# yurimjeon1892/EFGH

Hardware: AMD Instinct MI355X
Metric: frame-pairs/sec EFGHNet fwd+bwd (384x1280 RGB + 64x2048 range), whole job (higher is better)
Workload: dtype f32; 1 GPU; BASELINE.json configs[2]: EFGHNet fwd+bwd with efghloss + gradient all-reduce + fused Adam, synthetic 384x1280 RGB + 131072-point sweep, batch=8 per GPU, random-init weights; global_batch=8, points=131072, parallelism=dp1

## Files before the change

efgh_amd/csrc/wino.hip:

```cpp
#include "common.h"
#include <type_traits>


namespace {

typedef float f32x16 __attribute__((ext_vector_type(16)));

__device__ __attribute__((aligned(16))) float g_zero_page[16];

constexpr int TM = 64, TN = 64, KC = 16, LD = KC;

struct WinoArgs {
    const float *A; long long lda; int C;
    int B, H, W, TW;
    const float *U; int N;
    long long Mt;
    const float *bias, *scale, *shift, *residual; long long ldr;
    int act; float slope;
    float *out; long long ldo;
    float *stats;
    unsigned nbx;
    int smode;
    const float *bn_raw; long long bn_ldraw;
    const float *bn_y; long long bn_ldy;
    const float *bn_psc, *bn_psh, *bn_mean, *bn_invstd;
    int bn_act; float bn_slope;
};

template <bool BNM, bool HPOOL = false>
__global__ void __launch_bounds__(256, 2) k_wino43(const WinoArgs p) {
    __shared__ __attribute__((aligned(16))) float Vs[6 * TM * LD];
    __shared__ __attribute__((aligned(16))) float Us[6 * TN * LD];
    __shared__ long long tpix[TM];
    __shared__ int tcnt[TM];

    const int tid = threadIdx.x, lane = tid & 63, wave = tid >> 6;
    const int wm = wave >> 1, wn = wave & 1, l31 = lane & 31, lh = lane >> 5;
    const unsigned nbx = p.nbx, nblk = gridDim.x;
    const unsigned q8 = nblk >> 3, r8 = nblk & 7, xcd = blockIdx.x & 7, within = blockIdx.x >> 3;
    const unsigned lin = (xcd < r8 ? xcd * (q8 + 1) : r8 * (q8 + 1) + (xcd - r8) * q8) + within;
    const unsigned tile_m = lin / nbx, tile_n = lin - tile_m * nbx;
    const long long m0 = (long long)tile_m * TM;
    const int n0 = tile_n * TN;
    if (m0 >= p.Mt) return;

    const int st = tid >> 2, cq = (tid & 3) * 4;
    const int cqs = ((tid & 3) ^ ((st >> 2) & 3)) * 4;
    long long pix0 = 0;
    unsigned cmask = 0, rmask = 0;
    {
        const long long t = m0 + st;
        if (t < p.Mt) {
            const int xt = (int)(t % p.TW); const long long r = t / p.TW;
            const int y = (int)(r % p.H); const long long b = r / p.H;
            const int x0 = 4 * xt - 1;
#pragma unroll
            for (int q = 0; q < 6; ++q) if ((unsigned)(x0 + q) < (unsigned)p.W) cmask |= 1u << q;
#pragma unroll
            for (int kh = 0; kh < 3; ++kh) if ((unsigned)(y + kh - 1) < (unsigned)p.H) rmask |= 1u << kh;
            pix0 = (b * p.H + y) * p.W + x0;
        }
    }
    if (tid < TM) {
        const long long t = m0 + tid;
        long long o = -1; int cnt = 0;
        if (t < p.Mt) {
            const int xt = (int)(t % p.TW); const long long r = t / p.TW;
            o = r * p.W + 4 * xt;
            cnt = p.W - 4 * xt; cnt = cnt > 4 ? 4 : cnt;
            if (HPOOL) {
                const int wp = p.W >> 1;
                o = r * wp + 2 * xt;
                cnt = wp - 2 * xt; cnt = cnt > 2 ? 2 : cnt;
                if (cnt <= 0) { o = -1; cnt = 0; }
            }
        }
        tpix[tid] = o; tcnt[tid] = cnt;
    }
    const long long ustride = (long long)p.N * KC;
    const float *ubase = p.U + (long long)(n0 + st) * KC + cq;
// ... 48 lines not shown
                v4.e = q42 - q31;                                                                    \
                v5.e = 4.f * d1 - 5.f * d3 + d5;                                                     \
            }
            EFGH_BT(x) EFGH_BT(y) EFGH_BT(z) EFGH_BT(w)
#undef EFGH_BT
#define EFGH_ST(a, vv, uu)                                                                            \
            *reinterpret_cast<float4 *>(&Vs[(a * TM + st) * LD + cqs]) = vv;                         \
            *reinterpret_cast<float4 *>(&Us[(a * TN + st) * LD + cqs]) = uu;
            EFGH_ST(0, v0, ru0) EFGH_ST(1, v1, ru1) EFGH_ST(2, v2, ru2) EFGH_ST(3, v3, ru3) EFGH_ST(4, v4, ru4) EFGH_ST(5, v5, ru5)
#undef EFGH_ST
        }
        __syncthreads();
        const bool more = ch + 1 < nchunks;
        if (more) EFGH_CHUNK_ADDR(ch + 1)
        {
            const int sw = (l31 >> 2) & 3, q0 = ((2 * lh) ^ sw) * 4, q1 = ((2 * lh + 1) ^ sw) * 4;
            const float *va = &Vs[(wm * 32 + l31) * LD];
            const float *ub = &Us[(wn * 32 + l31) * LD];
            float4 fa[2][2], fb[2][2];
            fa[0][0] = *reinterpret_cast<const float4 *>(va + q0); fa[0][1] = *reinterpret_cast<const float4 *>(va + q1);
            fb[0][0] = *reinterpret_cast<const float4 *>(ub + q0); fb[0][1] = *reinterpret_cast<const float4 *>(ub + q1);
#pragma unroll
            for (int a = 0; a < 6; ++a) {
                const int cur = a & 1, nxt = cur ^ 1;
                if (a < 5) {
                    fa[nxt][0] = *reinterpret_cast<const float4 *>(va + (a + 1) * TM * LD + q0);
                    fa[nxt][1] = *reinterpret_cast<const float4 *>(va + (a + 1) * TM * LD + q1);
                    fb[nxt][0] = *reinterpret_cast<const float4 *>(ub + (a + 1) * TN * LD + q0);
                    fb[nxt][1] = *reinterpret_cast<const float4 *>(ub + (a + 1) * TN * LD + q1);
                }
                if (more) {
                    if (a == 0) EFGH_LOAD_PAIR(0, ra0, ru0)
                    if (a == 1) EFGH_LOAD_PAIR(1, ra1, ru1)
                    if (a == 2) EFGH_LOAD_PAIR(2, ra2, ru2)
                    if (a == 3) EFGH_LOAD_PAIR(3, ra3, ru3)
                    if (a == 4) EFGH_LOAD_PAIR(4, ra4, ru4)
                    if (a == 5) EFGH_LOAD_PAIR(5, ra5, ru5)
                }
                __builtin_amdgcn_sched_barrier(0);
                acc[a] = __builtin_amdgcn_mfma_f32_32x32x2f32(fa[cur][0].x, fb[cur][0].x, acc[a], 0, 0, 0);
                acc[a] = __builtin_amdgcn_mfma_f32_32x32x2f32(fa[cur][0].y, fb[cur][0].y, acc[a], 0, 0, 0);
                acc[a] = __builtin_amdgcn_mfma_f32_32x32x2f32(fa[cur][0].z, fb[cur][0].z, acc[a], 0, 0, 0);
                acc[a] = __builtin_amdgcn_mfma_f32_32x32x2f32(fa[cur][0].w, fb[cur][0].w, acc[a], 0, 0, 0);
                acc[a] = __builtin_amdgcn_mfma_f32_32x32x2f32(fa[cur][1].x, fb[cur][1].x, acc[a], 0, 0, 0);
                acc[a] = __builtin_amdgcn_mfma_f32_32x32x2f32(fa[cur][1].y, fb[cur][1].y, acc[a], 0, 0, 0);
                acc[a] = __builtin_amdgcn_mfma_f32_32x32x2f32(fa[cur][1].z, fb[cur][1].z, acc[a], 0, 0, 0);
                acc[a] = __builtin_amdgcn_mfma_f32_32x32x2f32(fa[cur][1].w, fb[cur][1].w, acc[a], 0, 0, 0);
                __builtin_amdgcn_sched_barrier(0);
            }
        }
        __syncthreads();
    }

    float *ssum = Vs, *ssq = Vs + 2 * TN;
    const int coll = wn * 32 + l31, col = n0 + coll;
    const float bi = p.bias ? p.bias[col] : 0.f;
    const float sc = p.scale ? p.scale[col] : 1.f;
    const float sf = p.shift ? p.shift[col] : 0.f;
    float s1 = 0.f, s2 = 0.f;
    constexpr bool bnm = BNM;
    float b_psc = 0.f, b_psh = 0.f, b_mu = 0.f, b_is = 0.f;
    if (bnm) {
        if (!p.bn_y) { b_psc = p.bn_psc[col]; b_psh = p.bn_psh[col]; }
        b_mu = p.bn_mean[col]; b_is = p.bn_invstd[col];
    }
    const float neg = p.act == 1 ? 0.f : (p.act == 2 ? p.slope : 1.f);
    auto rows = [&](auto res_c, auto full_c) {
        constexpr bool RES = decltype(res_c)::value, FULL = decltype(full_c)::value;
#pragma unroll
        for (int r = 0; r < 16; ++r) {
            const int rl = wm * 32 + (r & 3) + 8 * (r >> 2) + 4 * lh;
            const long long opix = tpix[rl];
            const int cnt = FULL ? 4 : tcnt[rl];
            if (!FULL && opix < 0) continue;
            float *op = p.out + opix * p.ldo + col;
            float rv[4] = {0.f, 0.f, 0.f, 0.f};
            if (RES) {
                const float *rp = p.residual + opix * p.ldr + col;
#pragma unroll
                for (int i = 0; i < 4; ++i) if (FULL || i < cnt) rv[i] = rp[i * p.ldr];
            }
            const float m0_ = acc[0][r], m1 = acc[1][r], m2 = acc[2][r], m3 = acc[3][r], m4 = acc[4][r], m5 = acc[5][r];
            const float s12 = m1 + m2, d12 = m1 - m2, s34 = m3 + m4, d34 = m3 - m4;
            const float yv[4] = {m0_ + s12 + s34, d12 + 2.f * d34, s12 + 4.f * s34, d12 + 8.f * d34 + m5};
            if (HPOOL) {
                float w[4];
#pragma unroll
                for (int i = 0; i < 4; ++i) { float v = yv[i] + bi; v = v * sc + sf; w[i] = act_neg(v, neg); }
                st_out(op, fmaxf(w[0], w[1]));
                if (FULL || cnt > 1) st_out(op + p.ldo, fmaxf(w[2], w[3]));
                continue;
            }
#pragma unroll
            for (int i = 0; i < 4; ++i) {
                if (!FULL && i >= cnt) continue;
                float v = yv[i] + bi;
                if (!bnm) { s1 += v; s2 = fmaf(v, v, s2); }
                v = v * sc + sf;
                if (RES) v += rv[i];
                v = act_neg(v, neg);
                st_out(op + i * p.ldo, v);
                if (bnm) {
                    const float rw = p.bn_raw[(opix + i) * p.bn_ldraw + col];
                    const float yy = p.bn_y ? p.bn_y[(opix + i) * p.bn_ldy + col] : rw * b_psc + b_psh;
                    const float g = p.bn_act == 1 ? (yy > 0.f ? v : 0.f) : p.bn_act == 2 ? (yy > 0.f ? v : v * p.bn_slope) : v;
                    s1 += g; s2 += g * ((rw - b_mu) * b_is);
                }
            }
        }
    };
    const bool full = m0 + TM <= p.Mt && (p.W & 3) == 0;
    if (p.residual) {
        if (full) rows(std::true_type{}, std::true_type{});
        else rows(std::true_type{}, std::false_type{});
    } else {
        if (full) rows(std::false_type{}, std::true_type{});
        else rows(std::false_type{}, std::false_type{});
    }
    if (p.stats) {
        s1 += __shfl_xor(s1, 32); s2 += __shfl_xor(s2, 32);
        if (lh == 0) { ssum[wm * TN + coll] = s1; ssq[wm * TN + coll] = s2; }
        __syncthreads();
        if (tid < TN) {
            p.stats[((long long)tile_m * 2 + 0) * p.N + n0 + tid] = ssum[tid] + ssum[TN + tid];
            p.stats[((long long)tile_m * 2 + 1) * p.N + n0 + tid] = ssq[tid] + ssq[TN + tid];
        }
    }
}

__global__ void k_wino_pack(const float *__restrict__ Wp, float *__restrict__ U, int N, int C) {
    const long long total = 3LL * C * N;
    for (long long i = (long long)blockIdx.x * blockDim.x + threadIdx.x; i < total; i += (long long)gridDim.x * blockDim.x)
        wino_pack_item(Wp, U, N, C, i);
}

constexpr int TT = 16;

struct WinoWArgs {
    const float *A; long long lda; int C;
    const float *G; long long ldg; int N;
    int B, H, W, TW;
    long long Mt; long long tchunk;
    float *S;
    unsigned kt, nt;
};

constexpr int WR_WAVES = 12;

__global__ void __launch_bounds__(64 * WR_WAVES, 1) k_wino_wgrad_rows(const WinoWArgs p, int strips, int chunks, int rh, int ct) {
    __shared__ __attribute__((aligned(16))) float Gs[6 * TT * 64];
    __shared__ __attribute__((aligned(16))) float Vr[3][6 * TT * 64];
    const int tid = threadIdx.x, lane = tid & 63, wave = __builtin_amdgcn_readfirstlane(tid >> 6);
    const int kg = wave >> 2, wn = (wave >> 1) & 1, wc = wave & 1, l31 = lane & 31, lh = lane >> 5;
    const int unit = blockIdx.x, strip = unit % strips, ur = unit / strips, chk = ur % chunks;
    const long long b = ur / chunks;
    const int y0 = chk * rh, y1 = y0 + rh < p.H ? y0 + rh : p.H;
    const int c0 = (blockIdx.y % ct) * 64, n0 = (blockIdx.y / ct) * 64;
    if (y0 >= y1) return;
    const int role = wave >> 2, st = tid & 255, ts = st >> 4, q4 = (st & 15) * 4;
    const int xt = strip * TT + ts, x0 = 4 * xt - 1, xg = 4 * xt;
    const bool tv = xt < p.TW;
    const float *zpage = g_zero_page;
    float4 r0, r1, r2, r3, r4, r5;
    auto load_x = [&](int r) {
        const bool rok = tv && (unsigned)r < (unsigned)p.H;
        const float *xrow = p.A + (((b * p.H + r) * p.W + x0) * p.lda + c0 + q4);
#define EFGH_LDX(q, dst) dst = *reinterpret_cast<const float4 *>((rok && (unsigned)(x0 + q) < (unsigned)p.W) ? xrow + (long long)q * p.lda : zpage);
        EFGH_LDX(0, r0) EFGH_LDX(1, r1) EFGH_LDX(2, r2) EFGH_LDX(3, r3) EFGH_LDX(4, r4) EFGH_LDX(5, r5)
#undef EFGH_LDX
    };
    auto load_g = [&](int r) {
        const float *grow = p.G + (((b * p.H + r) * p.W + xg) * p.ldg + n0 + q4);
#define EFGH_LDG(i, dst) dst = *reinterpret_cast<const float4 *>((tv && (xg + i) < p.W) ? grow + (long long)i * p.ldg : zpage);
        EFGH_LDG(0, r0) EFGH_LDG(1, r1) EFGH_LDG(2, r2) EFGH_LDG(3, r3)
#undef EFGH_LDG
    };
    auto stage_x = [&](float *V) {
        float4 v0, v1, v2, v3, v4, v5;
#define EFGH_TR(e)                                                                                    \
        {                                                                                            \
// ... 60 lines not shown
            for (int s8 = 0; s8 < 8; ++s8) { fg[0][s8] = gp[s8 * 128]; fv[0][s8] = vp[s8 * 128]; }
#pragma unroll
            for (int a = 0; a < 6; ++a) {
                const int cur = a & 1, nxt = cur ^ 1;
                if (a < 5) {
#pragma unroll
                    for (int s8 = 0; s8 < 8; ++s8) {
                        fg[nxt][s8] = gp[(a + 1) * TT * 64 + s8 * 128];
                        fv[nxt][s8] = vp[(a + 1) * TT * 64 + s8 * 128];
                    }
                }
#pragma unroll
                for (int s8 = 0; s8 < 8; ++s8)
                    acc[a] = __builtin_amdgcn_mfma_f32_32x32x2f32(fg[cur][s8], fv[cur][s8], acc[a], 0, 0, 0);
            }
        }
        __syncthreads();
        s0 = s0 == 2 ? 0 : s0 + 1;
    }
    const long long K3 = 3LL * p.C;
    float *sb = p.S + (((long long)unit * 3) * p.N + n0 + wn * 32) * K3 + kg * p.C + c0 + wc * 32 + l31;
    const long long plane = (long long)p.N * K3;
#pragma unroll
    for (int r = 0; r < 16; ++r) {
        const int nl = (r & 3) + 8 * (r >> 2) + 4 * lh;
        const float s0 = acc[0][r], s1 = acc[1][r], s2 = acc[2][r], s3 = acc[3][r], s4 = acc[4][r], s5 = acc[5][r];
        sb[nl * K3] = s0 + s1 + s2 + s3 + s4;
        sb[plane + nl * K3] = (s1 - s2) + 2.f * (s3 - s4);
        sb[2 * plane + nl * K3] = (s1 + s2) + 4.f * (s3 + s4) + s5;
    }
}

__global__ void k_wino_wgrad_finish3(const float *__restrict__ S, float *__restrict__ dWp, int N, int C, long long on, long long oc,
                                     long long ot, int Nr, int Cr, int accumulate) {
    const long long K3 = 3LL * C, total = (long long)N * K3;
    for (long long i = (long long)blockIdx.x * blockDim.x + threadIdx.x; i < total; i += (long long)gridDim.x * blockDim.x) {
        const int kc = (int)(i % K3); const long long n = i / K3;
        const int kh = kc / C, c = kc - kh * C;
        if (n >= Nr || c >= Cr) continue;
        float *o = dWp + n * on + c * oc + (kh * 3) * ot;
        if (accumulate) { o[0] += S[i]; o[ot] += S[total + i]; o[2 * ot] += S[2 * total + i]; }
        else { o[0] = S[i]; o[ot] = S[total + i]; o[2 * ot] = S[2 * total + i]; }
    }
}

bool supported(const efgh_gemm_desc *d) {
    if (!d || d->mode != 1 || d->T != 9 || d->C % KC || d->N % TN || d->M_dev || d->nbatch > 1) return false;
    if (d->sh != 1 || d->sw != 1 || d->osh != 1 || d->osw != 1 || d->oh0 || d->ow0) return false;
    if (d->Hv != d->Hin || d->Wv != d->Win || d->Ho != d->Hin || d->Wo != d->Win) return false;
    for (int t = 0; t < 9; ++t) if (d->dh[t] != t / 3 - 1 || d->dw[t] != t % 3 - 1) return false;
    return d->lda % 4 == 0;
}

}

extern "C" int efgh_wino_supported(const efgh_gemm_desc *d) { return supported(d) ? 1 : 0; }

extern "C" int32_t efgh_wino_grid_m(int32_t B, int32_t H, int32_t W) {
    const long long mt = (long long)B * H * ((W + 3) / 4);
    return (int32_t)((mt + TM - 1) / TM);
}

extern "C" int efgh_wino_pack(const float *Wp, float *U, int32_t N, int32_t C, void *stream_) {
    EFGH_CHECK_ARG(Wp && U && N > 0 && C > 0 && C % KC == 0);
    const long long total = 3LL * C * N;
    long long g = (total + 255) / 256;
    k_wino_pack<<<(int)(g > 8192 ? 8192 : g), 256, 0, (hipStream_t)stream_>>>(Wp, U, N, C);
    EFGH_CHECK_LAUNCH();
    return EFGH_OK;
}

extern "C" int efgh_wino_conv3x3(const efgh_gemm_desc *d, const float *U, void *stream_) {
    EFGH_CHECK_ARG(supported(d) && U && d->A && d->out);
    EFGH_CHECK_ARG((((uintptr_t)d->A) & 15) == 0 && (((uintptr_t)U) & 15) == 0);
    EFGH_CHECK_ARG(d->B > 0 && d->M == (int64_t)d->B * d->Hin * d->Win);
    WinoArgs a;
    a.A = d->A; a.lda = d->lda; a.C = d->C;
    a.B = d->B; a.H = d->Hin; a.W = d->Win; a.TW = (d->Win + 3) / 4;
    a.U = U; a.N = d->N; a.Mt = (long long)d->B * d->Hin * a.TW;
    a.bias = d->bias; a.scale = d->scale; a.shift = d->shift; a.residual = d->residual; a.ldr = d->ldr;
    a.act = d->act; a.slope = d->slope; a.out = d->out; a.ldo = d->ldo; a.stats = d->stats;
    a.smode = d->stats ? d->stats_mode : 0;
    if (a.smode == 1) EFGH_CHECK_ARG(d->bn_raw && d->bn_mean && d->bn_invstd && (d->bn_y || (d->bn_pscale && d->bn_pshift)));
    a.bn_raw = d->bn_raw; a.bn_ldraw = d->bn_ldraw; a.bn_y = d->bn_y; a.bn_ldy = d->bn_ldy;
    a.bn_psc = d->bn_pscale; a.bn_psh = d->bn_pshift; a.bn_mean = d->bn_mean; a.bn_invstd = d->bn_invstd;
    a.bn_act = d->bn_act; a.bn_slope = d->bn_slope;
    a.nbx = (unsigned)(d->N / TN);
    const long long nby = (a.Mt + TM - 1) / TM;
    EFGH_CHECK_ARG(a.nbx * nby < 0x7fffffffLL);
    if (a.smode == 1) k_wino43<true><<<(unsigned)(a.nbx * nby), 256, 0, (hipStream_t)stream_>>>(a);
    else k_wino43<false><<<(unsigned)(a.nbx * nby), 256, 0, (hipStream_t)stream_>>>(a);
    EFGH_CHECK_LAUNCH();
    return EFGH_OK;
}

extern "C" int efgh_wino_conv3x3_hpool(const efgh_gemm_desc *d, const float *U, void *stream_) {
    EFGH_CHECK_ARG(supported(d) && U && d->A && d->out && !d->residual && !d->stats && d->Win >= 2);
    EFGH_CHECK_ARG((((uintptr_t)d->A) & 15) == 0 && (((uintptr_t)U) & 15) == 0);
    EFGH_CHECK_ARG(d->B > 0 && d->M == (int64_t)d->B * d->Hin * d->Win);
    WinoArgs a;
    a.A = d->A; a.lda = d->lda; a.C = d->C;
    a.B = d->B; a.H = d->Hin; a.W = d->Win; a.TW = (d->Win + 3) / 4;
    a.U = U; a.N = d->N; a.Mt = (long long)d->B * d->Hin * a.TW;
    a.bias = d->bias; a.scale = d->scale; a.shift = d->shift; a.residual = nullptr; a.ldr = 0;
    a.act = d->act; a.slope = d->slope; a.out = d->out; a.ldo = d->ldo; a.stats = nullptr; a.smode = 0;
    a.bn_raw = nullptr; a.bn_ldraw = 0; a.bn_y = nullptr; a.bn_ldy = 0;
    a.bn_psc = a.bn_psh = a.bn_mean = a.bn_invstd = nullptr; a.bn_act = 0; a.bn_slope = 0.f;
    a.nbx = (unsigned)(d->N / TN);
    const long long nby = (a.Mt + TM - 1) / TM;
    EFGH_CHECK_ARG(a.nbx * nby < 0x7fffffffLL);
    k_wino43<false, true><<<(unsigned)(a.nbx * nby), 256, 0, (hipStream_t)stream_>>>(a);
    EFGH_CHECK_LAUNCH();
    return EFGH_OK;
}

extern "C" int efgh_wino_wgrad_supported(const efgh_gemm_desc *d) {
    return (supported(d) && d->C % 64 == 0) ? 1 : 0;
}

static long long wino_wgrad_row_units(const efgh_gemm_desc *d, int *strips_out, int *chunks_out, int *rh_out) {
    const int strips = ((d->Win + 3) / 4 + TT - 1) / TT, blocks = (d->C / 64) * (d->N / 64);
    int best = 1; double beste = -1.0;
    for (int c = 1; c <= 8; ++c) {
        const int rh = (d->Hin + c - 1) / c;
        if (c > 1 && rh < 8) break;
        const long long wg = (long long)d->B * strips * ((d->Hin + rh - 1) / rh) * blocks;
        const double eff = (double)wg / (double)(((wg + 255) / 256) * 256) * (double)rh / (double)(rh + 2);
        if (eff > beste + 1e-9) { beste = eff; best = c; }
    }
    const int rh = (d->Hin + best - 1) / best, chunks = (d->Hin + rh - 1) / rh;
    if (strips_out) *strips_out = strips;
    if (chunks_out) *chunks_out = chunks;
    if (rh_out) *rh_out = rh;
    return (long long)d->B * strips * chunks;
}

extern "C" int64_t efgh_wino_wgrad_workspace(const efgh_gemm_desc *d) {
    if (!supported(d) || d->C % 64 != 0 || d->B <= 0) return 0;
    return wino_wgrad_row_units(d, nullptr, nullptr, nullptr) * 3 * (int64_t)d->N * 3 * d->C;
}

extern "C" int efgh_wino_wgrad(const efgh_gemm_desc *d, const float *G, int64_t ldg, float *S, float *dWp,
                               const efgh_wgrad_out_desc *out, void *stream_) {
    hipStream_t st = (hipStream_t)stream_;
    EFGH_CHECK_ARG(supported(d) && d->C % 64 == 0 && d->A && G && S && dWp && ldg % 4 == 0);
    EFGH_CHECK_ARG((((uintptr_t)d->A) & 15) == 0 && (((uintptr_t)G) & 15) == 0);
    EFGH_CHECK_ARG(d->B > 0 && d->M == (int64_t)d->B * d->Hin * d->Win);
    WinoWArgs a;
    a.A = d->A; a.lda = d->lda; a.C = d->C; a.G = G; a.ldg = ldg; a.N = d->N;
    a.B = d->B; a.H = d->Hin; a.W = d->Win; a.TW = (d->Win + 3) / 4;
    a.Mt = (long long)d->B * d->Hin * a.TW;
    a.S = S;
    const int kt = 3 * d->C / 64, nt = d->N / 64;
    int strips = 0, chunks = 0, rh = 0;
    const long long zs = wino_wgrad_row_units(d, &strips, &chunks, &rh);
    EFGH_CHECK_ARG(zs < 0x7fffffffLL && (long long)(d->C / 64) * nt < 65536);
    a.tchunk = 0; a.kt = (unsigned)kt; a.nt = (unsigned)nt;
    k_wino_wgrad_rows<<<dim3((unsigned)zs, (unsigned)((d->C / 64) * nt)), 64 * WR_WAVES, 0, st>>>(a, strips, chunks, rh, d->C / 64);
    EFGH_CHECK_LAUNCH();
    if (zs > 1) efgh_launch_fold_splits(S, (int)zs, 3LL * d->N * 3 * d->C, S, st);
    const long long total = (long long)d->N * 3 * d->C;
    long long g = (total + 255) / 256;
    const bool direct = efgh_wgrad_out_fits(out, d->N, 9, d->C);
    if (direct)
// ... 7 lines not shown
```

efgh_amd/ops.py:

```python
import ctypes
import os as _os
import threading
import weakref

import torch

from . import _C
from ._C import c_float, c_int32, c_int64, ptr

ACT_NONE, ACT_RELU, ACT_LEAKY = 0, 1, 2


def _L():
    return _C.lib()


def _st():
    return _C.stream_ptr()


def ceil4(n):
    return (n + 3) // 4 * 4


# ... 571 lines not shown
    d = _desc(A, lda, C, T, mode, N, M, geom, table, a_off, Wp, out, ldo, out_off, bias, scale, shift, residual, ldr, res_off, act, slope,
              stats, M_dev, batch)
    d.table_alias_mask = 1 if (alias_mask and mode == 2) else 0
    if route == 'sc' and not _sc_aligned(d, lda, ldo, residual, ldr, stats):
        route = gemm_route(*key, aligned=False)
    if pool and route not in ('c4', 'wino2d', 'wino_hpool'):
        raise _C.EfghError('gather_gemm(pool=True) on a launch no pooling epilogue serves (ask pool_fusable() first)')
    ev = _prof_start(PROFILE)
    bn_stats = None
    if route == 'thin':
        if TRACE_THIN is not None:
            TRACE_THIN.append(int(_L().efgh_thin_supported(ctypes.byref(d))))
        _C.check(_L().efgh_thin_gemm(ctypes.byref(d), _st()))
    elif route == 'c4':
        assert lda % 4 == 0
        _C.check((_L().efgh_c4_conv3x3_pooled if pool else _L().efgh_c4_conv3x3)(ctypes.byref(d), _st()))
    elif route == 'sc':
        _C.check(_L().efgh_sc_conv3x3(ctypes.byref(d), _st()))
    elif route == 'wino2d':
        if (bn_bwd is not None and stats is None and BN_BWD_FUSED_2D and out_off == 0 and not pool and bn_bwd.fits(M, N)
                and bn_bwd.y is None and bn_bwd.raw.stride(-2) % 4 == 0):
            rows = _L().efgh_wino2d_stats_rows(c_int32(geom[0]), c_int32(geom[1]), c_int32(geom[2]), c_int32(N))
            bn_stats = _bn_bwd_sums(d, bn_bwd, rows, N, out.device)
        _wino2d_forward(d, A, a_off, lda, C, N, geom, Wp, pool=pool, lazy=lazy, pre_v=pre_v)
    elif route == 'wino_hpool':
        _C.check(_L().efgh_wino_conv3x3_hpool(ctypes.byref(d), ptr(wino_weight(Wp, N, C)), _st()))
    elif route == 'wino':
        if bn_bwd is not None and stats is None and BN_BWD_FUSED and out_off == 0 and bn_bwd.fits(M, N):
            rows = _L().efgh_wino_grid_m(c_int32(geom[0]), c_int32(geom[1]), c_int32(geom[2]))
            bn_stats = _bn_bwd_sums(d, bn_bwd, rows, N, out.device)
        _C.check(_L().efgh_wino_conv3x3(ctypes.byref(d), ptr(wino_weight(Wp, N, C)), _st()))
    else:
        _C.check(_L().efgh_gather_gemm(ctypes.byref(d), _st()))
    if ev is not None:
        _prof_end(ev, route, (mode, M, N, T, C), float(flops) if flops is not None else 2.0 * M * N * T * C, PROFILE, PROFILE_WINO,
                  batched=batch is not None)
    return bn_stats


def _bn_bwd_sums(d, src, rows, N, device):
    part = torch.empty((rows, 2, N), dtype=torch.float32, device=device)
    d.stats, d.stats_mode = part.data_ptr(), 1
    d.bn_raw, d.bn_ldraw = src.raw.data_ptr(), src.raw.stride(-2)
    if src.y is not None:
        d.bn_y, d.bn_ldy = src.y.data_ptr(), src.y.stride(-2)
    else:
        d.bn_pscale, d.bn_pshift = src.psc.data_ptr(), src.psh.data_ptr()
    d.bn_mean, d.bn_invstd = src.mean.data_ptr(), src.invstd.data_ptr()
    d.bn_act, d.bn_slope = src.act, src.slope
    return part


GEMM_DMA = True


def apply_switches():
    _L().efgh_gather_gemm_set_dma(c_int32(1 if GEMM_DMA else 0))


PLANE_DMA = True
PLANE_DMA_NBUF = 0
PROFILE_WINO2D = None
PROFILE_WINO2D_GEMM = None
PLANES_SPLIT = None
PLANE_SPLIT_HITS = [0, 0]


def planes_split_active():
    if PLANES_SPLIT is not None:
        return bool(PLANES_SPLIT)
    return torch.backends.cuda.matmul.fp32_precision == 'tf32'


def _planes_split_now():
    m = TLS.planes_split
    return planes_split_active() if m is None else m


def _batched_plain_gemm(A3, W3, out3, rows, C, N):
    g = _desc(A3, 36 * C, C, 1, 0, N, rows, Wp=W3, out=out3, ldo=36 * N, batch=(36, C, N * C, N))
    ev = _prof_start(PROFILE_WINO2D_GEMM)
    if PLANE_DMA and _L().efgh_plane_gemm_supported(ctypes.byref(g)):
        if _planes_split_now():
            PLANE_SPLIT_HITS[0] += 1
            _C.check(_L().efgh_plane_gemm_x6(ctypes.byref(g), c_int32(PLANE_DMA_NBUF), _st()))
        else:
            _C.check(_L().efgh_plane_gemm(ctypes.byref(g), c_int32(PLANE_DMA_NBUF), _st()))
    else:
        _C.check(_L().efgh_gather_gemm(ctypes.byref(g), _st()))
    _prof_end(ev, 'planes', (0, rows, N, 36, C), 2.0 * 36 * rows * C * N, PROFILE_WINO2D_GEMM)


W2V_CACHE = {}
W2V_KEEP = True


def w2v_clear():
    me = threading.get_ident()
    with _LOCK:
        for k in [k for k, v in W2V_CACHE.items() if v[2] == me]:
            del W2V_CACHE[k]


POOL_FUSED = True
POOL_HALF = True


def pool_fusable(mode, C, N, geom, residual=None, stats=None):
    if not (POOL_FUSED and residual is None and stats is None and geom is not None and geom[1] >= 2 and geom[2] >= 2):
        return False
# ... 868 lines not shown
```

include/efgh_hip.h:

```cpp
#ifndef EFGH_HIP_H
#define EFGH_HIP_H
#include <stdint.h>

#ifdef __cplusplus
extern "C" {
#endif

#define EFGH_OK 0
#define EFGH_E_INVALID (-1)
#define EFGH_E_LAUNCH (-2)
#define EFGH_WROTE_OUT 1

const char *efgh_last_error(void);

#define EFGH_ABI_VERSION 4
int efgh_version(void);

#define EFGH_LATTICE_INFO_H 0
#define EFGH_LATTICE_INFO_ERR 1
#define EFGH_LATTICE_INFO_ALIAS 2
#define EFGH_LATTICE_INFO_CURSOR 3
#define EFGH_LATTICE_INFO_SEG 4
#define EFGH_LATTICE_MAX_SAMPLES 1024

// ... 287 lines not shown
int32_t efgh_sc_stats_rows(int32_t B, int32_t H, int32_t W);
int efgh_sc_conv3x3(const efgh_gemm_desc *d, void *stream);
int efgh_sc_wgrad_supported(const efgh_gemm_desc *d);
int64_t efgh_sc_wgrad_workspace(const efgh_gemm_desc *d);
int efgh_sc_wgrad(const efgh_gemm_desc *d, const float *G, int64_t ldg, float *dWp, float *workspace,
                  const efgh_wgrad_out_desc *out, void *stream);
int efgh_c4_supported(const efgh_gemm_desc *d);
int32_t efgh_c4_stats_rows(int32_t B, int32_t Ho, int32_t Wo);
int efgh_c4_conv3x3(const efgh_gemm_desc *d, void *stream);
int efgh_c4_pooled_supported(const efgh_gemm_desc *d);
int efgh_c4_conv3x3_pooled(const efgh_gemm_desc *d, void *stream);
int efgh_c4_wgrad_supported(const efgh_gemm_desc *d);
int64_t efgh_c4_wgrad_workspace(const efgh_gemm_desc *d);
int efgh_c4_wgrad(const efgh_gemm_desc *d, const float *G, int64_t ldg, float *dWp, float *workspace,
                  const efgh_wgrad_out_desc *out, void *stream);

int efgh_debug_occupancy(char *out, int32_t cap);

int efgh_gather_gemm_set_dma(int32_t on);

int efgh_plane_gemm_supported(const efgh_gemm_desc *d);
int efgh_plane_gemm(const efgh_gemm_desc *d, int32_t nbuf, void *stream);
int efgh_plane_wgrad_supported(const efgh_gemm_desc *d, int64_t ldg);
int64_t efgh_plane_wgrad_workspace(const efgh_gemm_desc *d);
int efgh_plane_wgrad_batched(const efgh_gemm_desc *d, const float *G, int64_t ldg, int64_t batch_stride_g, float *dWp,
                             int64_t batch_stride_dw, float *workspace, int32_t nbuf, void *stream);

int efgh_plane_gemm_x6(const efgh_gemm_desc *d, int32_t nbuf, void *stream);
int efgh_plane_wgrad_x6_batched(const efgh_gemm_desc *d, const float *G, int64_t ldg, int64_t batch_stride_g, float *dWp,
                                int64_t batch_stride_dw, float *workspace, int32_t nbuf, void *stream);

int efgh_convt_col2im(const float *Y, int64_t ldy, int32_t B, int32_t Hin, int32_t Win, int32_t Ho, int32_t Wo,
                      int32_t O, int32_t pad, const float *scale, const float *shift, int32_t act, float slope,
                      float *out, int64_t ldo, void *stream);
int efgh_convt_im2col(const float *G, int64_t ldg, int32_t B, int32_t Hin, int32_t Win, int32_t Ho, int32_t Wo,
                      int32_t O, int32_t pad, float *Ycol, int64_t ldy, void *stream);

int efgh_corr_pack_cam(const float *cam, const float *cam_mm, int32_t B, int32_t h, int32_t wc, int32_t segw,
                       int32_t nseg, int32_t nsplit, float *Wc, void *stream);
int efgh_corr_fold(const float *P, int32_t B, int32_t nsplit, int64_t Mv, int32_t ldp, int32_t nseg, int32_t segw,
                   int32_t nj, float *logit, float *score, void *stream);
int efgh_norm_bwd(const float *x, const float *dxn, const float *mm, int32_t B, int64_t n, float *part, float *dx, void *stream);
int efgh_corr_planes(const float *x, const float *mm, int32_t B, int32_t h, int32_t w, int32_t w_in_pitch, int32_t wP,
                     float *out, void *stream);
int efgh_corr_unplanes(const float *in, int32_t B, int32_t h, int32_t w, int32_t wP, float *out, void *stream);
int efgh_corr_toeplitz(const float *dl, int32_t B, int32_t nj, int32_t rows, int32_t cols, int32_t colsP, int32_t transpose,
                       float *T, void *stream);

int efgh_wino_supported(const efgh_gemm_desc *d);
int32_t efgh_wino_grid_m(int32_t B, int32_t H, int32_t W);
int efgh_wino_pack(const float *Wp, float *U, int32_t N, int32_t C, void *stream);
int efgh_wino_conv3x3_hpool(const efgh_gemm_desc *d, const float *U, void *stream);
int efgh_wino_conv3x3(const efgh_gemm_desc *d, const float *U, void *stream);
int efgh_wino_wgrad_supported(const efgh_gemm_desc *d);
int64_t efgh_wino_wgrad_workspace(const efgh_gemm_desc *d);
int efgh_wino_wgrad(const efgh_gemm_desc *d, const float *G, int64_t ldg, float *S, float *dWp, const efgh_wgrad_out_desc *out,
                    void *stream);

int efgh_prep_affine_nearest_u8(const uint8_t *in, int32_t h, int32_t w, const int64_t *coef6_host, uint8_t *out,
                                int32_t nh, int32_t nw, void *stream);
int efgh_prep_crop_pad_u8(const uint8_t *in, int32_t h, int32_t w, int32_t oy, int32_t ox, uint8_t *out, int32_t th,
                          int32_t tw, void *stream);
int efgh_prep_resample_u8(const uint8_t *in, int32_t h, int32_t w, int32_t axis, int32_t out_size, const int32_t *bounds,
                          const int32_t *coeffs, int32_t ksize, uint8_t *out, void *stream);
int efgh_prep_hwc_to_chw_u8(const uint8_t *in, int32_t h, int32_t w, uint8_t *chw, uint8_t *mask, void *stream);
int efgh_prep_u8_to_f32_chw_pad(const uint8_t *in, int32_t h, int32_t w, int32_t oy, int32_t ox, float *out, int32_t th,
                                int32_t tw, void *stream);
int32_t efgh_prep_filter_blocks(int32_t n);
int efgh_prep_radius_filter(const float *pcd, const int32_t *pre_idx, int32_t n, int32_t flip_xy, float radius,
                            int32_t *block_scratch, int32_t *keep_idx, int32_t *count, void *stream);
int efgh_prep_gather_transform(const float *pcd, const int32_t *keep_idx, const int32_t *sel, int32_t n_sel,
                               int32_t flip_xy, const double *T34, int32_t num_points, float *out32, double *out64,
                               void *stream);

int efgh_pose_errors(const float *gt, const float *pred, int32_t B, int32_t mode, float *rot_err, float *trs_err,
                     void *stream);

int32_t efgh_gimg_loss_groups(int64_t n);
int efgh_gimg_loss_fwd(const float *pred_depth, const float *pred_mask, int64_t mask_bstride, const float *gdep4,
                       const uint8_t *img_mask, int32_t B, int64_t HW, float *gt_depth, float *gt_mask, double *part,
                       float *out3, void *stream);
int efgh_gimg_loss_bwd(const float *pred_depth, const float *pred_mask, int64_t mask_bstride, const float *gt_depth,
                       const uint8_t *img_mask, int32_t B, int64_t HW, const float *sums3, const float *g_depth,
                       const float *g_mask, float *d_pred_depth, float *d_pred_mask, int64_t dmask_bstride, void *stream);

int efgh_sum_depth_last(const float *pc, int64_t pc_cstride, int32_t N, const double *T34, int32_t H, int32_t W, int32_t *idx_ws,
                        uint8_t *out, void *stream);
int efgh_sum_range_last(const float *pc, int64_t pc_cstride, int32_t N, const double *T34, int32_t H, int32_t W, double fov_up,
                        double fov_down, int32_t *idx_ws, double *out, void *stream);
int efgh_sum_paint(const void *jobs_dev, int32_t njobs, void *stream);
int efgh_sum_colorize(const double *minmax, int64_t n, const uint8_t *lut, uint8_t *rgb, uint8_t *mask, void *stream);

int efgh_pose_head_normal(const float *abs_logits, int64_t lda, const float *sgn_logits, int64_t lds, int32_t B, int32_t nd,
                          float dx, float dy, float dz, float *abs_out, float *normal, float *R44, void *stream);
int efgh_pose_head_yaw(const float *score, int64_t lds, int32_t B, int32_t n, float *R44, void *stream);
int efgh_pose_cam_T_velo(const float *c_T, int64_t ldc, const float *l_T, const float *calib, const float *A, int32_t B,
                         float *out34, void *stream);

int efgh_pose_head_normal_bwd(const float *abs_logits, int64_t lda, const float *sgn_logits, int64_t lds, int32_t B, int32_t nd,
                              float dx, float dy, float dz, const float *g_abs, const float *g_normal, const float *g_R44,
                              float *g_abs_logits, void *stream);
int efgh_pose_mat44_mul(const float *a, const float *b, int32_t B, int32_t transpose_a, int32_t transpose_b, float *out, void *stream);
int efgh_pose_rotation_between(const float *src3, int32_t B, float dx, float dy, float dz, float *R44, void *stream);
int efgh_pose_cam_T_velo_bwd(const float *c_T, int64_t ldc, const float *l_T, const float *calib, const float *A,
                             const float *g_out34, int32_t B, float *g_cT33, float *g_lT44, void *stream);

// ... 20 lines not shown
```

Baseline: 31.37 frame-pairs/s.

## Add row-block Winograd F(4,3) conv kernel reusing input rows across kernel heights

```diff
diff --git a/efgh_amd/csrc/wino.hip b/efgh_amd/csrc/wino.hip
--- a/efgh_amd/csrc/wino.hip
+++ b/efgh_amd/csrc/wino.hip
@@ -26,6 +26,86 @@
     const float *bn_psc, *bn_psh, *bn_mean, *bn_invstd;
     int bn_act; float bn_slope;
 };
+
+template <bool BNM, bool HPOOL>
+__device__ __forceinline__ void wino43_epilogue(const WinoArgs &p, const f32x16 (&acc)[6], float *scratch, const long long *tpix,
+                                                const int *tcnt, unsigned tile_m, int n0, bool full) {
+    const int tid = threadIdx.x, lane = tid & 63, wave = tid >> 6;
+    const int wm = wave >> 1, wn = wave & 1, l31 = lane & 31, lh = lane >> 5;
+    float *ssum = scratch, *ssq = scratch + 2 * TN;
+    const int coll = wn * 32 + l31, col = n0 + coll;
+    const float bi = p.bias ? p.bias[col] : 0.f;
+    const float sc = p.scale ? p.scale[col] : 1.f;
+    const float sf = p.shift ? p.shift[col] : 0.f;
+    float s1 = 0.f, s2 = 0.f;
+    constexpr bool bnm = BNM;
+    float b_psc = 0.f, b_psh = 0.f, b_mu = 0.f, b_is = 0.f;
+    if (bnm) {
+        if (!p.bn_y) { b_psc = p.bn_psc[col]; b_psh = p.bn_psh[col]; }
+        b_mu = p.bn_mean[col]; b_is = p.bn_invstd[col];
+    }
+    const float neg = p.act == 1 ? 0.f : (p.act == 2 ? p.slope : 1.f);
+    auto rows = [&](auto res_c, auto full_c) {
+        constexpr bool RES = decltype(res_c)::value, FULL = decltype(full_c)::value;
+#pragma unroll
+        for (int r = 0; r < 16; ++r) {
+            const int rl = wm * 32 + (r & 3) + 8 * (r >> 2) + 4 * lh;
+            const long long opix = tpix[rl];
+            const int cnt = FULL ? 4 : tcnt[rl];
+            if (!FULL && opix < 0) continue;
+            float *op = p.out + opix * p.ldo + col;
+            float rv[4] = {0.f, 0.f, 0.f, 0.f};
+            if (RES) {
+                const float *rp = p.residual + opix * p.ldr + col;
+#pragma unroll
+                for (int i = 0; i < 4; ++i) if (FULL || i < cnt) rv[i] = rp[i * p.ldr];
+            }
+            const float m0_ = acc[0][r], m1 = acc[1][r], m2 = acc[2][r], m3 = acc[3][r], m4 = acc[4][r], m5 = acc[5][r];
+            const float s12 = m1 + m2, d12 = m1 - m2, s34 = m3 + m4, d34 = m3 - m4;
+            const float yv[4] = {m0_ + s12 + s34, d12 + 2.f * d34, s12 + 4.f * s34, d12 + 8.f * d34 + m5};
+            if (HPOOL) {
+                float w[4];
+#pragma unroll
+                for (int i = 0; i < 4; ++i) { float v = yv[i] + bi; v = v * sc + sf; w[i] = act_neg(v, neg); }
+                st_out(op, fmaxf(w[0], w[1]));
+                if (FULL || cnt > 1) st_out(op + p.ldo, fmaxf(w[2], w[3]));
+                continue;
+            }
+#pragma unroll
+            for (int i = 0; i < 4; ++i) {
+                if (!FULL && i >= cnt) continue;
+                float v = yv[i] + bi;
+                if (!bnm) { s1 += v; s2 = fmaf(v, v, s2); }
+                v = v * sc + sf;
+                if (RES) v += rv[i];
+                v = act_neg(v, neg);
+                st_out(op + i * p.ldo, v);
+                if (bnm) {
+                    const float rw = p.bn_raw[(opix + i) * p.bn_ldraw + col];
+                    const float yy = p.bn_y ? p.bn_y[(opix + i) * p.bn_ldy + col] : rw * b_psc + b_psh;
+                    const float g = p.bn_act == 1 ? (yy > 0.f ? v : 0.f) : p.bn_act == 2 ? (yy > 0.f ? v : v * p.bn_slope) : v;
+                    s1 += g; s2 += g * ((rw - b_mu) * b_is);
+                }
+            }
+        }
+    };
+    if (p.residual) {
+        if (full) rows(std::true_type{}, std::true_type{});
+        else rows(std::true_type{}, std::false_type{});
+    } else {
+        if (full) rows(std::false_type{}, std::true_type{});
+        else rows(std::false_type{}, std::false_type{});
+    }
+    if (p.stats) {
+        s1 += __shfl_xor(s1, 32); s2 += __shfl_xor(s2, 32);
+        if (lh == 0) { ssum[wm * TN + coll] = s1; ssq[wm * TN + coll] = s2; }
+        __syncthreads();
+        if (tid < TN) {
+            p.stats[((long long)tile_m * 2 + 0) * p.N + n0 + tid] = ssum[tid] + ssum[TN + tid];
+            p.stats[((long long)tile_m * 2 + 1) * p.N + n0 + tid] = ssq[tid] + ssq[TN + tid];
+        }
+    }
+}
 
 template <bool BNM, bool HPOOL = false>
 __global__ void __launch_bounds__(256, 2) k_wino43(const WinoArgs p) {
@@ -180,80 +260,186 @@
         __syncthreads();
     }
 
-    float *ssum = Vs, *ssq = Vs + 2 * TN;
-    const int coll = wn * 32 + l31, col = n0 + coll;
-    const float bi = p.bias ? p.bias[col] : 0.f;
-    const float sc = p.scale ? p.scale[col] : 1.f;
-    const float sf = p.shift ? p.shift[col] : 0.f;
-    float s1 = 0.f, s2 = 0.f;
-    constexpr bool bnm = BNM;
-    float b_psc = 0.f, b_psh = 0.f, b_mu = 0.f, b_is = 0.f;
-    if (bnm) {
-        if (!p.bn_y) { b_psc = p.bn_psc[col]; b_psh = p.bn_psh[col]; }
-        b_mu = p.bn_mean[col]; b_is = p.bn_invstd[col];
-    }
-    const float neg = p.act == 1 ? 0.f : (p.act == 2 ? p.slope : 1.f);
-    auto rows = [&](auto res_c, auto full_c) {
-        constexpr bool RES = decltype(res_c)::value, FULL = decltype(full_c)::value;
-#pragma unroll
-        for (int r = 0; r < 16; ++r) {
-            const int rl = wm * 32 + (r & 3) + 8 * (r >> 2) + 4 * lh;
-            const long long opix = tpix[rl];
-            const int cnt = FULL ? 4 : tcnt[rl];
-            if (!FULL && opix < 0) continue;
-            float *op = p.out + opix * p.ldo + col;
-            float rv[4] = {0.f, 0.f, 0.f, 0.f};
-            if (RES) {
-                const float *rp = p.residual + opix * p.ldr + col;
-#pragma unroll
-                for (int i = 0; i < 4; ++i) if (FULL || i < cnt) rv[i] = rp[i * p.ldr];
-            }
-            const float m0_ = acc[0][r], m1 = acc[1][r], m2 = acc[2][r], m3 = acc[3][r], m4 = acc[4][r], m5 = acc[5][r];
-            const float s12 = m1 + m2, d12 = m1 - m2, s34 = m3 + m4, d34 = m3 - m4;
-            const float yv[4] = {m0_ + s12 + s34, d12 + 2.f * d34, s12 + 4.f * s34, d12 + 8.f * d34 + m5};
-            if (HPOOL) {
-                float w[4];
-#pragma unroll
-                for (int i = 0; i < 4; ++i) { float v = yv[i] + bi; v = v * sc + sf; w[i] = act_neg(v, neg); }
-                st_out(op, fmaxf(w[0], w[1]));
-                if (FULL || cnt > 1) st_out(op + p.ldo, fmaxf(w[2], w[3]));
-                continue;
-            }
-#pragma unroll
-            for (int i = 0; i < 4; ++i) {
-                if (!FULL && i >= cnt) continue;
-                float v = yv[i] + bi;
-                if (!bnm) { s1 += v; s2 = fmaf(v, v, s2); }
-                v = v * sc + sf;
-                if (RES) v += rv[i];
-                v = act_neg(v, neg);
-                st_out(op + i * p.ldo, v);
-                if (bnm) {
-                    const float rw = p.bn_raw[(opix + i) * p.bn_ldraw + col];
-                    const float yy = p.bn_y ? p.bn_y[(opix + i) * p.bn_ldy + col] : rw * b_psc + b_psh;
-                    const float g = p.bn_act == 1 ? (yy > 0.f ? v : 0.f) : p.bn_act == 2 ? (yy > 0.f ? v : v * p.bn_slope) : v;
-                    s1 += g; s2 += g * ((rw - b_mu) * b_is);
+    wino43_epilogue<BNM, HPOOL>(p, acc, Vs, tpix, tcnt, tile_m, n0, m0 + TM <= p.Mt && (p.W & 3) == 0);
+}
+
+__device__ __forceinline__ void wino43_bt(const float4 &r0, const float4 &r1, const float4 &r2, const float4 &r3, const float4 &r4,
+                                          const float4 &r5, float4 &v0, float4 &v1, float4 &v2, float4 &v3, float4 &v4, float4 &v5) {
+#define EFGH_BT(e)                                                                                   \
+    {                                                                                                \
+        const float d0 = r0.e, d1 = r1.e, d2 = r2.e, d3 = r3.e, d4 = r4.e, d5 = r5.e;                  \
+        const float p42 = d4 - 4.f * d2, p31 = d3 - 4.f * d1;                                        \
+        const float q42 = d4 - d2, q31 = 2.f * (d3 - d1);                                            \
+        v0.e = 4.f * d0 - 5.f * d2 + d4;                                                             \
+        v1.e = p42 + p31;                                                                            \
+        v2.e = p42 - p31;                                                                            \
+        v3.e = q42 + q31;                                                                            \
+        v4.e = q42 - q31;                                                                            \
+        v5.e = 4.f * d1 - 5.f * d3 + d5;                                                             \
+    }
+    EFGH_BT(x) EFGH_BT(y) EFGH_BT(z) EFGH_BT(w)
+#undef EFGH_BT
+}
+
+template <int R, int TX>
+constexpr size_t wino_rows_lds() { return (size_t)(6 * (R + 2) * TX * LD + 6 * TN * LD) * sizeof(float) + TM * (sizeof(long long) + sizeof(int)); }
+
+template <int R, int TX, bool BNM, bool HPOOL = false>
+__global__ void __launch_bounds__(256, 2) k_wino43_rows(const WinoArgs p) {
+    constexpr int NV = (R + 2) * TX;
+    constexpr bool HALF = NV - TM < TM;
+    static_assert(R * TX == TM && TX % 16 == 0 && (NV - TM == TM || NV - TM == TM / 2), "row-block shape");
+    extern __shared__ __attribute__((aligned(16))) float wino_rows_smem[];
+    float *Vs = wino_rows_smem, *Us = Vs + 6 * NV * LD;
+    long long *tpix = reinterpret_cast<long long *>(Us + 6 * TN * LD);
+    int *tcnt = reinterpret_cast<int *>(tpix + TM);
+
+    const int tid = threadIdx.x, lane = tid & 63, wave = tid >> 6;
+    const int wm = wave >> 1, wn = wave & 1, l31 = lane & 31, lh = lane >> 5;
+    const unsigned nbx = p.nbx, nblk = gridDim.x;
+    const unsigned q8 = nblk >> 3, r8 = nblk & 7, xcd = blockIdx.x & 7, within = blockIdx.x >> 3;
+    const unsigned lin = (xcd < r8 ? xcd * (q8 + 1) : r8 * (q8 + 1) + (xcd - r8) * q8) + within;
+    const unsigned tile_m = lin / nbx, tile_n = lin - tile_m * nbx;
+    const int n0 = tile_n * TN;
+    const unsigned xbn = (unsigned)p.TW / TX, rbn = (unsigned)p.H / R;
+    const unsigned xb = tile_m % xbn, rb = tile_m / xbn;
+    const unsigned b = rb / rbn;
+    if (b >= (unsigned)p.B) return;
+    const int y0 = (int)(rb - b * rbn) * R, xt0 = (int)xb * TX;
+
+    if (tid < TM) {
+        const int xt = xt0 + tid % TX;
+        const long long r = (long long)b * p.H + y0 + tid / TX;
+        long long o = r * p.W + 4 * xt;
+        int cnt = p.W - 4 * xt; cnt = cnt > 4 ? 4 : cnt;
+        if (HPOOL) {
+            const int wp = p.W >> 1;
+            o = r * wp + 2 * xt;
+            cnt = wp - 2 * xt; cnt = cnt > 2 ? 2 : cnt;
+            if (cnt <= 0) { o = -1; cnt = 0; }
+        }
+        tpix[tid] = o; tcnt[tid] = cnt;
+    }
+
+    const int st = tid >> 2, cq = (tid & 3) * 4;
+    const int s1 = TM + (HALF ? (tid & 127) >> 2 : st);
+    const int cqs0 = ((tid & 3) ^ ((st >> 2) & 3)) * 4, cqs1 = ((tid & 3) ^ ((s1 >> 2) & 3)) * 4;
+    const float *zpage = g_zero_page;
+    unsigned cm0 = 0, cm1 = 0;
+    const float *a0p, *a1p;
+    {
+        auto item = [&](int s, unsigned &cm) -> const float * {
+            const int yy = y0 - 1 + s / TX, x0 = 4 * (xt0 + s % TX) - 1;
+            const bool rok = (unsigned)yy < (unsigned)p.H;
+            if (rok) {
+#pragma unroll
+                for (int q = 0; q < 6; ++q) if ((unsigned)(x0 + q) < (unsigned)p.W) cm |= 1u << q;
+            }
+            const int yc = rok ? yy : y0;
+            return p.A + ((((long long)b * p.H + yc) * p.W + x0) * p.lda + cq);
+        };
+        a0p = item(st, cm0);
+        a1p = item(s1, cm1);
+    }
+    const long long ustride = (long long)p.N * KC;
+    const float *urow = p.U + (long long)(n0 + st) * KC + cq;
+
+    float4 ra0, ra1, ra2, ra3, ra4, ra5, ru0, ru1, ru2, ru3, ru4, ru5;
+#define EFGH_RLDP(q, dst, base, cm)                                                                   \
+    dst = *reinterpret_cast<const float4 *>(((cm >> q) & 1u) ? base + (long long)q * p.lda : zpage);
+#define EFGH_RLDU(q, dst) dst = *reinterpret_cast<const float4 *>(urow + q * ustride);
+#define EFGH_RSTV(s, cqs)                                                                             \
+    {                                                                                                \
+        float4 v0, v1, v2, v3, v4, v5;                                                               \
+        wino43_bt(ra0, ra1, ra2, ra3, ra4, ra5, v0, v1, v2, v3, v4, v5);                             \
+        *reinterpret_cast<float4 *>(&Vs[(0 * NV + s) * LD + cqs]) = v0;                              \
+        *reinterpret_cast<float4 *>(&Vs[(1 * NV + s) * LD + cqs]) = v1;                              \
+        *reinterpret_cast<float4 *>(&Vs[(2 * NV + s) * LD + cqs]) = v2;                              \
+        *reinterpret_cast<float4 *>(&Vs[(3 * NV + s) * LD + cqs]) = v3;                              \
+        *reinterpret_cast<float4 *>(&Vs[(4 * NV + s) * LD + cqs]) = v4;                              \
+        *reinterpret_cast<float4 *>(&Vs[(5 * NV + s) * LD + cqs]) = v5;                              \
+    }
+
+    f32x16 acc[6];
+#pragma unroll
+    for (int a = 0; a < 6; ++a)
+#pragma unroll
+        for (int r = 0; r < 16; ++r) acc[a][r] = 0.f;
+
+    const int ccn = p.C / KC;
+    EFGH_RLDP(0, ra0, a0p, cm0) EFGH_RLDP(1, ra1, a0p, cm0) EFGH_RLDP(2, ra2, a0p, cm0)
+    EFGH_RLDP(3, ra3, a0p, cm0) EFGH_RLDP(4, ra4, a0p, cm0) EFGH_RLDP(5, ra5, a0p, cm0)
+    EFGH_RLDU(0, ru0) EFGH_RLDU(1, ru1) EFGH_RLDU(2, ru2) EFGH_RLDU(3, ru3) EFGH_RLDU(4, ru4) EFGH_RLDU(5, ru5)
+    const int sw = (l31 >> 2) & 3, q0 = ((2 * lh) ^ sw) * 4, q1 = ((2 * lh + 1) ^ sw) * 4;
+    const float *ub = &Us[(wn * 32 + l31) * LD];
+    for (int cc = 0; cc < ccn; ++cc) {
+        const bool last = cc + 1 == ccn;
+        const bool it1 = !HALF || (wave >> 1) == (cc & 1);
+        EFGH_RSTV(st, cqs0)
+#pragma unroll
+        for (int kh = 0; kh < 3; ++kh) {
+            if (kh == 1 && it1) EFGH_RSTV(s1, cqs1)
+            *reinterpret_cast<float4 *>(&Us[(0 * TN + st) * LD + cqs0]) = ru0;
+            *reinterpret_cast<float4 *>(&Us[(1 * TN + st) * LD + cqs0]) = ru1;
+            *reinterpret_cast<float4 *>(&Us[(2 * TN + st) * LD + cqs0]) = ru2;
+            *reinterpret_cast<float4 *>(&Us[(3 * TN + st) * LD + cqs0]) = ru3;
+            *reinterpret_cast<float4 *>(&Us[(4 * TN + st) * LD + cqs0]) = ru4;
+            *reinterpret_cast<float4 *>(&Us[(5 * TN + st) * LD + cqs0]) = ru5;
+            __syncthreads();
+            const bool more_u = !(last && kh == 2);
+            const bool more_p = kh == 0 ? it1 : (kh == 1 && !last);
+            const float *pb = kh == 0 ? a1p : a0p + KC;
+            const unsigned pm = kh == 0 ? cm1 : cm0;
+            if (more_u) urow += 6 * ustride;
+            const float *va = &Vs[(wm * 32 + l31 + kh * TX) * LD];
+            float4 fa[2][2], fb[2][2];
+            fa[0][0] = *reinterpret_cast<const float4 *>(va + q0); fa[0][1] = *reinterpret_cast<const float4 *>(va + q1);
+            fb[0][0] = *reinterpret_cast<const float4 *>(ub + q0); fb[0][1] = *reinterpret_cast<const float4 *>(ub + q1);
+#pragma unroll
+            for (int a = 0; a < 6; ++a) {
+                const int cur = a & 1, nxt = cur ^ 1;
+                if (a < 5) {
+                    fa[nxt][0] = *reinterpret_cast<const float4 *>(va + (a + 1) * NV * LD + q0);
+                    fa[nxt][1] = *reinterpret_cast<const float4 *>(va + (a + 1) * NV * LD + q1);
+                    fb[nxt][0] = *reinterpret_cast<const float4 *>(ub + (a + 1) * TN * LD + q0);
+                    fb[nxt][1] = *reinterpret_cast<const float4 *>(ub + (a + 1) * TN * LD + q1);
                 }
-            }
-        }
-    };
-    const bool full = m0 + TM <= p.Mt && (p.W & 3) == 0;
-    if (p.residual) {
-        if (full) rows(std::true_type{}, std::true_type{});
-        else rows(std::true_type{}, std::false_type{});
-    } else {
-        if (full) rows(std::false_type{}, std::true_type{});
-        else rows(std::false_type{}, std::false_type{});
-    }
-    if (p.stats) {
-        s1 += __shfl_xor(s1, 32); s2 += __shfl_xor(s2, 32);
-        if (lh == 0) { ssum[wm * TN + coll] = s1; ssq[wm * TN + coll] = s2; }
-        __syncthreads();
-        if (tid < TN) {
-            p.stats[((long long)tile_m * 2 + 0) * p.N + n0 + tid] = ssum[tid] + ssum[TN + tid];
-            p.stats[((long long)tile_m * 2 + 1) * p.N + n0 + tid] = ssq[tid] + ssq[TN + tid];
-        }
-    }
+                if (more_u) {
+                    if (a == 0) EFGH_RLDU(0, ru0)
+                    if (a == 1) EFGH_RLDU(1, ru1)
+                    if (a == 2) EFGH_RLDU(2, ru2)
+                    if (a == 3) EFGH_RLDU(3, ru3)
+                    if (a == 4) EFGH_RLDU(4, ru4)
+                    if (a == 5) EFGH_RLDU(5, ru5)
+                }
+                if (kh < 2 && more_p) {
+                    if (a == 0) EFGH_RLDP(0, ra0, pb, pm)
+                    if (a == 1) EFGH_RLDP(1, ra1, pb, pm)
+                    if (a == 2) EFGH_RLDP(2, ra2, pb, pm)
+                    if (a == 3) EFGH_RLDP(3, ra3, pb, pm)
+                    if (a == 4) EFGH_RLDP(4, ra4, pb, pm)
+                    if (a == 5) EFGH_RLDP(5, ra5, pb, pm)
+                }
+                __builtin_amdgcn_sched_barrier(0);
+                acc[a] = __builtin_amdgcn_mfma_f32_32x32x2f32(fa[cur][0].x, fb[cur][0].x, acc[a], 0, 0, 0);
+                acc[a] = __builtin_amdgcn_mfma_f32_32x32x2f32(fa[cur][0].y, fb[cur][0].y, acc[a], 0, 0, 0);
+                acc[a] = __builtin_amdgcn_mfma_f32_32x32x2f32(fa[cur][0].z, fb[cur][0].z, acc[a], 0, 0, 0);
+                acc[a] = __builtin_amdgcn_mfma_f32_32x32x2f32(fa[cur][0].w, fb[cur][0].w, acc[a], 0, 0, 0);
+                acc[a] = __builtin_amdgcn_mfma_f32_32x32x2f32(fa[cur][1].x, fb[cur][1].x, acc[a], 0, 0, 0);
+                acc[a] = __builtin_amdgcn_mfma_f32_32x32x2f32(fa[cur][1].y, fb[cur][1].y, acc[a], 0, 0, 0);
+                acc[a] = __builtin_amdgcn_mfma_f32_32x32x2f32(fa[cur][1].z, fb[cur][1].z, acc[a], 0, 0, 0);
+                acc[a] = __builtin_amdgcn_mfma_f32_32x32x2f32(fa[cur][1].w, fb[cur][1].w, acc[a], 0, 0, 0);
+                __builtin_amdgcn_sched_barrier(0);
+            }
+            __syncthreads();
+        }
+        a0p += KC; a1p += KC;
+    }
+#undef EFGH_RLDP
+#undef EFGH_RLDU
+#undef EFGH_RSTV
+
+    wino43_epilogue<BNM, HPOOL>(p, acc, Vs, tpix, tcnt, tile_m, n0, (p.W & 3) == 0);
 }
 
 __global__ void k_wino_pack(const float *__restrict__ Wp, float *__restrict__ U, int N, int C) {
@@ -420,7 +606,49 @@
     return d->lda % 4 == 0;
 }
 
-}
+int g_wino_rows = 1;
+
+int wino_rows_plan(int H, int W) {
+    const int tw = (W + 3) / 4;
+    const bool f4 = H > 0 && H % 4 == 0 && tw % 16 == 0, f2 = H > 0 && H % 2 == 0 && tw % 32 == 0;
+    if (g_wino_rows == 0) return 0;
+    if (g_wino_rows == 2) return f2 ? 2 : 0;
+    if (g_wino_rows == 4) return f4 ? 4 : 0;
+    return f2 ? 2 : (f4 ? 4 : 0);
+}
+
+std::atomic<unsigned long long> g_rows_raised[6];
+
+template <int R, int TX, bool BNM, bool HPOOL>
+int wino_launch_rows(const WinoArgs &a, long long nby, hipStream_t st) {
+    constexpr size_t lds = wino_rows_lds<R, TX>();
+    static_assert(lds <= 80 * 1024, "two workgroups per CU");
+    if (!efgh_raise_lds_once(g_rows_raised[(R == 4) * 3 + (BNM ? 1 : HPOOL ? 2 : 0)], (const void *)k_wino43_rows<R, TX, BNM, HPOOL>, (int)lds)) {
+        efgh_set_error("%s:%d: cannot raise the dynamic LDS limit of k_wino43_rows", __FILE__, __LINE__);
+        return EFGH_E_LAUNCH;
+    }
+    k_wino43_rows<R, TX, BNM, HPOOL><<<(unsigned)(a.nbx * nby), 256, lds, st>>>(a);
+    return EFGH_OK;
+}
+
+template <bool BNM, bool HPOOL>
+int wino_launch(const WinoArgs &a, long long nby, hipStream_t st) {
+    const int r = wino_rows_plan(a.H, a.W);
+    if (r == 4) return wino_launch_rows<4, 16, BNM, HPOOL>(a, nby, st);
+    if (r == 2) return wino_launch_rows<2, 32, BNM, HPOOL>(a, nby, st);
+    k_wino43<BNM, HPOOL><<<(unsigned)(a.nbx * nby), 256, 0, st>>>(a);
+    return EFGH_OK;
+}
+
+}
+
+extern "C" int efgh_wino_set_rows(int32_t mode) {
+    const int old = g_wino_rows;
+    if (mode == 0 || mode == 1 || mode == 2 || mode == 4) g_wino_rows = mode;
+    return old;
+}
+
+extern "C" int32_t efgh_wino_rows_plan(int32_t H, int32_t W) { return wino_rows_plan(H, W); }
 
 extern "C" int efgh_wino_supported(const efgh_gemm_desc *d) { return supported(d) ? 1 : 0; }
 
@@ -456,8 +684,8 @@
     a.nbx = (unsigned)(d->N / TN);
     const long long nby = (a.Mt + TM - 1) / TM;
     EFGH_CHECK_ARG(a.nbx * nby < 0x7fffffffLL);
-    if (a.smode == 1) k_wino43<true><<<(unsigned)(a.nbx * nby), 256, 0, (hipStream_t)stream_>>>(a);
-    else k_wino43<false><<<(unsigned)(a.nbx * nby), 256, 0, (hipStream_t)stream_>>>(a);
+    const int rc = a.smode == 1 ? wino_launch<true, false>(a, nby, (hipStream_t)stream_) : wino_launch<false, false>(a, nby, (hipStream_t)stream_);
+    if (rc != EFGH_OK) return rc;
     EFGH_CHECK_LAUNCH();
     return EFGH_OK;
 }
@@ -477,7 +705,8 @@
     a.nbx = (unsigned)(d->N / TN);
     const long long nby = (a.Mt + TM - 1) / TM;
     EFGH_CHECK_ARG(a.nbx * nby < 0x7fffffffLL);
-    k_wino43<false, true><<<(unsigned)(a.nbx * nby), 256, 0, (hipStream_t)stream_>>>(a);
+    const int rc = wino_launch<false, true>(a, nby, (hipStream_t)stream_);
+    if (rc != EFGH_OK) return rc;
     EFGH_CHECK_LAUNCH();
     return EFGH_OK;
 }
diff --git a/efgh_amd/ops.py b/efgh_amd/ops.py
--- a/efgh_amd/ops.py
+++ b/efgh_amd/ops.py
@@ -647,10 +647,12 @@
 
 
 GEMM_DMA = True
+WINO_ROWS = 1
 
 
 def apply_switches():
     _L().efgh_gather_gemm_set_dma(c_int32(1 if GEMM_DMA else 0))
+    _L().efgh_wino_set_rows(c_int32(int(WINO_ROWS)))
 
 
 PLANE_DMA = True
diff --git a/include/efgh_hip.h b/include/efgh_hip.h
--- a/include/efgh_hip.h
+++ b/include/efgh_hip.h
@@ -363,6 +363,8 @@
 int efgh_wino_pack(const float *Wp, float *U, int32_t N, int32_t C, void *stream);
 int efgh_wino_conv3x3_hpool(const efgh_gemm_desc *d, const float *U, void *stream);
 int efgh_wino_conv3x3(const efgh_gemm_desc *d, const float *U, void *stream);
+int efgh_wino_set_rows(int32_t mode);
+int32_t efgh_wino_rows_plan(int32_t H, int32_t W);
 int efgh_wino_wgrad_supported(const efgh_gemm_desc *d);
 int64_t efgh_wino_wgrad_workspace(const efgh_gemm_desc *d);
 int efgh_wino_wgrad(const efgh_gemm_desc *d, const float *G, int64_t ldg, float *S, float *dWp, const efgh_wgrad_out_desc *out,
```

New measurement: 31.47 frame-pairs/s, median of 2. No clear change (+0.3%).
